# hellojialee/Improved-Body-Parts

Measured on AMD Instinct MI355X. Metric: fps_512_infer, higher is better.
Workload: dtype bf16; 1 GPU; model=4-stage IMHN @512x512, mode=infer, global_batch=4, input=512, parallelism=dp1

## Files before the change

### improved_body_parts_amd/models/layers.py

```python
from __future__ import annotations

import torch
import torch.nn.functional as F
from torch import nn

from .. import ops

LEAKY_SLOPE = 0.01


class Conv(nn.Module):

    def __init__(self, inp_dim, out_dim, kernel_size=3, stride=1, bn=True, relu=True,
                 dropout=False, dialated=1):
        super().__init__()
        self.inp_dim = inp_dim
        self.dropout = dropout
        self.relu = nn.LeakyReLU(negative_slope=LEAKY_SLOPE, inplace=True) if relu else None
        pad = (kernel_size - 1) // 2
        if bn:
            self.conv = nn.Conv2d(inp_dim, out_dim, kernel_size, stride, padding=pad, bias=False)
            self.bn = nn.BatchNorm2d(out_dim)
        else:
            self.conv = nn.Conv2d(inp_dim, out_dim, kernel_size, stride, padding=pad, bias=True)
# ... 76 lines not shown
        )
        if ins != outs:
            self.skipConv = nn.Sequential(
                nn.Conv2d(ins, outs, 1, bias=False),
                nn.BatchNorm2d(outs),
            )
        self.relu = nn.LeakyReLU(negative_slope=LEAKY_SLOPE, inplace=True)
        self.ins = ins
        self.outs = outs

    def forward(self, x):
        cb = self.convBlock
        y = ops.conv_bn_act(x, cb[0], cb[1], act=True, training=self.training)
        y = ops.conv_bn_act(y, cb[3], cb[4], act=True, training=self.training)
        if self.ins != self.outs:
            residual = ops.conv_bn_act(x, self.skipConv[0], self.skipConv[1], act=False,
                                       training=self.training)
        else:
            residual = x
        return ops.conv_bn_add_act(y, cb[6], cb[7], residual, act=self.relu_flag,
                                   training=self.training)


class BasicResidual(nn.Module):

    def __init__(self, inp_dim, out_dim, stride=1, bn=True, relu=True):
        super().__init__()
        self.relu_flag = relu
        self.conv1 = nn.Conv2d(inp_dim, out_dim, 3, padding=1, stride=stride, bias=False)
        self.bn1 = nn.BatchNorm2d(out_dim)
        self.relu1 = nn.LeakyReLU(negative_slope=LEAKY_SLOPE, inplace=True)
        self.conv2 = nn.Conv2d(out_dim, out_dim, 3, padding=1, bias=False)
        self.bn2 = nn.BatchNorm2d(out_dim)
        self.skip = nn.Sequential(
            nn.Conv2d(inp_dim, out_dim, 1, stride=stride, bias=False),
# ... 115 lines not shown
```

### improved_body_parts_amd/ops/__init__.py

```python
from __future__ import annotations

import os

import torch
import torch.nn.functional as F

from . import _backend
from ._backend import (
    hip_available,
    hip_extension,
    require_hip,
    use_hip_for,
)

LEAKY_SLOPE = 0.01



def conv_bn_act(x, conv, bn, act: bool, training: bool,
                residual_post=None, residual_post2=None):
    if use_hip_for(x):
        from . import conv as _conv
        return _conv.conv_bn_act_hip(x, conv, bn, act=act, residual=None,
                                     training=training,
# ... 27 lines not shown
                    residual_post=None):
    if use_hip_for(x):
        from . import conv as _conv
        return _conv.conv_bn_act_hip(x, conv, bn, act=act, residual=residual,
                                     training=training,
                                     residual_post=residual_post)
    y = conv(x)
    if bn is not None:
        y = bn(y)
    y = y + residual
    if act:
        y = F.leaky_relu(y, LEAKY_SLOPE, inplace=True)
    if residual_post is not None:
        y = y + residual_post
    return y


def conv_bn_act_group(items):
    if items and all(use_hip_for(it["x"]) for it in items):
        from . import conv as _conv
        return _conv.conv_bn_act_group_hip(items)
    out = []
    for it in items:
        if it.get("residual") is not None:
            y = conv_bn_add_act(
                it["x"], it["conv"], it["bn"], it["residual"], act=it["act"],
                training=it.get("training", False),
                residual_post=it.get("residual_post"))
            if it.get("residual_post2") is not None:
                y = y + it["residual_post2"]
# ... 105 lines not shown
```

### improved_body_parts_amd/ops/conv.py

```python
from __future__ import annotations

import os

import torch
import torch.nn.functional as F

from . import conv_kernels
from ._backend import hip_extension
from ._cache import versioned

LEAKY_SLOPE = 0.01
_CL = torch.channels_last


def _to_cl(t):
    return t.contiguous(memory_format=_CL)


def _conv_forward(x, weight, bias, stride, padding, dilation):
    y = conv_kernels.conv_fwd(x, weight, stride, padding, dilation)
    if y is None:
        y = F.conv2d(x, weight, None, stride, padding, dilation)
        y = _to_cl(y)
    if bias is not None:
# ... 220 lines not shown
def upsample_conv_bn_act_hip(low, conv, bn, act: bool, training: bool = False,
                             residual_post=None, residual_post2=None):
    if _on_inference_path(low, bn, training) and upconv_fold_enabled():
        if conv_kernels.upfold_supported(low, conv.weight, conv.stride,
                                         conv.padding, conv.dilation):
            scale, shift = _inference_epilogue(conv, bn)
            return conv_kernels.upfold_fwd(
                _to_cl(low), conv.weight, scale=scale, shift=shift, act=act,
                residual_post=residual_post, residual_post2=residual_post2)
    from . import spatial
    return conv_bn_act_hip(spatial.upsample2x_hip(low), conv, bn, act=act,
                           training=training, residual_post=residual_post,
                           residual_post2=residual_post2)


def conv_group_enabled() -> bool:
    return os.environ.get("IBP_CONV_GROUP", "1") != "0"


def conv_bn_act_group_hip(items):
    if len(items) > 1 and conv_group_enabled() and all(
            _on_inference_path(it["x"], it["bn"], it.get("training", False))
            for it in items):
        members = []
        for it in items:
            conv = it["conv"]
            scale, shift = _inference_epilogue(conv, it["bn"])
            members.append(dict(
                x=_to_cl(it["x"]), weight=conv.weight, stride=conv.stride,
                padding=conv.padding, dilation=conv.dilation, scale=scale,
# ... 13 lines not shown
```

### improved_body_parts_amd/ops/conv_kernels.py

```python
from __future__ import annotations

import os

import torch

from ._backend import hip_extension
from ._cache import versioned

_CL = torch.channels_last

DISABLE = os.environ.get("IBP_AMD_DISABLE_MFMA_CONV") == "1"


def _supported(x, stride):
    return not DISABLE and x.dtype == torch.bfloat16 \
        and stride[0] == stride[1]


def _cl(t):
    return None if t is None else t.contiguous(memory_format=_CL)


_NO_EPI = (None, None, None, False, None, None)

# ... 207 lines not shown
    cout = weight.shape[0]
    post = []
    for r in (residual_post, residual_post2):
        if r is not None:
            assert tuple(r.shape) == (n, cout, 2 * h, 2 * w_), \
                f"residual {tuple(r.shape)} is not the upsampled output shape"
            r = _cl(r).permute(0, 2, 3, 1)
        post.append(r)
    geom = [n, h, w_, cin, cout, 3, 3, 1, 1, 1, 1, 1, 2 * h, 2 * w_, 1]
    y = hip_extension().conv_mfma_upfold_fwd(
        x.permute(0, 2, 3, 1), upfold_packed_weight(weight), geom, scale,
        shift, act, *post)
    return y.permute(0, 3, 1, 2)


def conv_dgrad(dy, weight, x_shape, stride, padding, dilation):
    if not _supported(dy, stride):
        return None
    cout, _, kh, kw = weight.shape
    pad = (dilation[0] * (kh - 1) - padding[0],
           dilation[1] * (kw - 1) - padding[1])
    if pad[0] < 0 or pad[1] < 0:
        return None
    dx = hip_extension().conv_mfma_fwd(*_conv_args(
        dy, packed_weight_dgrad(weight), (x_shape[1], cout, kh, kw), (1, 1),
        pad, dilation, zs=stride[0], out_hw=x_shape[2:]))
    return dx.permute(0, 3, 1, 2)


def conv_wgrad(x, dy, w_shape, stride, padding, dilation):
# ... 6 lines not shown
```

### improved_body_parts_amd/ops/csrc/bindings.cpp

```cpp
#include <torch/extension.h>

using torch::Tensor;

std::vector<int64_t> bn_v8_geometry(int64_t M, int64_t C);
std::vector<Tensor> bn_stats(const Tensor& x_mc, int64_t C);
std::vector<Tensor> bn_finalize(
    const Tensor& sums, const Tensor& sumsq, int64_t M, const Tensor& gamma,
    const Tensor& beta, const c10::optional<Tensor>& running_mean,
    const c10::optional<Tensor>& running_var,
    const c10::optional<Tensor>& num_batches, double momentum, double eps);
std::vector<Tensor> bn_stats_finalize(
    const Tensor& x_mc, int64_t C, const Tensor& gamma, const Tensor& beta,
    const c10::optional<Tensor>& running_mean,
    const c10::optional<Tensor>& running_var,
    const c10::optional<Tensor>& num_batches, double momentum, double eps);
Tensor bn_act_fwd(const Tensor& x, const Tensor& scale, const Tensor& shift,
                  const c10::optional<Tensor>& residual, double slope, bool act);
std::vector<Tensor> bn_act_bwd(const Tensor& dy, const Tensor& y, const Tensor& x,
                               const c10::optional<Tensor>& mean,
                               const c10::optional<Tensor>& invstd,
                               double slope, bool act, bool need_xhat, int64_t C);
Tensor bn_act_bwd_apply(const Tensor& dpre, const Tensor& x, const Tensor& mean,
                        const Tensor& invstd, const Tensor& gamma,
                        const c10::optional<Tensor>& sum_dpre,
// ... 21 lines not shown

Tensor focal_l2_fwd(const Tensor& pred, const Tensor& gt, const Tensor& mask,
                    int64_t heat_start, int64_t bkg_start, int64_t gamma,
                    double mtw, double ktw, double alpha, double beta);
Tensor focal_l2_bwd(const Tensor& pred, const Tensor& gt, const Tensor& mask,
                    const Tensor& stack_gscale, int64_t heat_start,
                    int64_t bkg_start, int64_t gamma, double mtw, double ktw,
                    double alpha, double beta);

Tensor conv_mfma_fwd(const Tensor& x, const Tensor& w_packed,
                     const std::vector<int64_t>& geom,
                     const c10::optional<Tensor>& scale,
                     const c10::optional<Tensor>& shift,
                     const c10::optional<Tensor>& residual, bool act,
                     const c10::optional<Tensor>& residual_post,
                     const c10::optional<Tensor>& residual_post2);

std::vector<Tensor> conv_mfma_fwd_grouped(
    const std::vector<Tensor>& xs, const std::vector<Tensor>& ws_packed,
    const std::vector<std::vector<int64_t>>& geom,
    const std::vector<c10::optional<Tensor>>& scales,
    const std::vector<c10::optional<Tensor>>& shifts,
    const std::vector<c10::optional<Tensor>>& residuals,
    const std::vector<bool>& acts,
    const std::vector<c10::optional<Tensor>>& residual_posts,
    const std::vector<c10::optional<Tensor>>& residual_post2s);

std::vector<int64_t> conv_mfma_tile_plan(int64_t M, int64_t Cout, int64_t K);

void pack_conv_weight(const Tensor& w, Tensor& fwd_pack,
                      const c10::optional<Tensor>& dgrad_pack);

void pack_upfold_weight(const Tensor& w, Tensor& out);
Tensor conv_mfma_upfold_fwd(const Tensor& x_low, const Tensor& packs,
                            const std::vector<int64_t>& geom,
                            const c10::optional<Tensor>& scale,
                            const c10::optional<Tensor>& shift, bool act,
                            const c10::optional<Tensor>& residual_post,
                            const c10::optional<Tensor>& residual_post2);
std::vector<int64_t> conv_mfma_upfold_plan(int64_t M_low, int64_t Cout,
                                           int64_t Cin);

Tensor conv_mfma_wgrad(const Tensor& x, const Tensor& dy, int64_t N, int64_t H,
                       int64_t W, int64_t Cin, int64_t Cout, int64_t KH,
                       int64_t KW, int64_t stride, int64_t pad_h, int64_t pad_w,
                       int64_t dil_h, int64_t dil_w, int64_t Ho, int64_t Wo);
std::vector<int64_t> conv_wgrad_plan(int64_t M, int64_t Cin, int64_t Cout,
                                     int64_t KH, int64_t KW);
// ... 44 lines not shown
  m.def("upsample2x_bwd", &upsample2x_bwd);
  m.def("se_reduce", &se_reduce);
  m.def("se_scale", &se_scale);
  m.def("se_gate", &se_gate, "fused GAP-gate: sigmoid(W2@leaky(W1@p+b1)+b2)",
        py::arg("pooled"), py::arg("w1"), py::arg("b1"), py::arg("w2"),
        py::arg("b2"), py::arg("slope"), py::arg("pool_scale") = 1.0);
  m.def("se_layer_grouped", &se_layer_grouped,
        "inference SE layers of independent maps: one launch per stage");
  m.def("focal_l2_fwd", &focal_l2_fwd);
  m.def("focal_l2_bwd", &focal_l2_bwd);
  m.def("conv_mfma_fwd", &conv_mfma_fwd, "MFMA implicit-GEMM conv forward",
        py::arg("x"), py::arg("w_packed"), py::arg("geom"),
        py::arg("scale") = c10::nullopt, py::arg("shift") = c10::nullopt,
        py::arg("residual") = c10::nullopt, py::arg("act") = false,
        py::arg("residual_post") = c10::nullopt,
        py::arg("residual_post2") = c10::nullopt);
  m.def("conv_mfma_fwd_grouped", &conv_mfma_fwd_grouped,
        "independent MFMA convs in one grouped launch per 8 (+ one combine)",
        py::arg("xs"), py::arg("ws_packed"), py::arg("geom"),
        py::arg("scales"), py::arg("shifts"), py::arg("residuals"),
        py::arg("acts"), py::arg("residual_posts"),
        py::arg("residual_post2s"));
  m.def("conv_mfma_tile_plan", &conv_mfma_tile_plan,
        "debug: [BM, BN, splitk, deep] planned for GEMM extents (M, Cout, K)",
        py::arg("M"), py::arg("Cout"), py::arg("K"));
  m.def("pack_conv_weight", &pack_conv_weight,
        "fwd + dgrad weight packs in one kernel",
        py::arg("w"), py::arg("fwd_pack"), py::arg("dgrad_pack") = c10::nullopt);
  m.def("pack_upfold_weight", &pack_upfold_weight,
        "3x3 weight -> four folded 2x2 packs [4][Cout][4*Cin] (nearest-x2 "
        "upsample folded into the conv)",
        py::arg("w"), py::arg("out"));
  m.def("conv_mfma_upfold_fwd", &conv_mfma_upfold_fwd,
        "conv3x3(nearest_x2(x_low)) + epilogue as four parity 2x2 convs in "
        "one grouped launch",
        py::arg("x_low"), py::arg("packs"), py::arg("geom"),
        py::arg("scale") = c10::nullopt, py::arg("shift") = c10::nullopt,
        py::arg("act") = false, py::arg("residual_post") = c10::nullopt,
        py::arg("residual_post2") = c10::nullopt);
  m.def("conv_mfma_upfold_plan", &conv_mfma_upfold_plan,
        "debug: [BM, BN, splitk, deep] shared by the four parities of an "
        "upfold conv over M_low low-resolution pixels",
        py::arg("M_low"), py::arg("Cout"), py::arg("Cin"));
  m.def("conv_mfma_wgrad", &conv_mfma_wgrad,
        "MFMA implicit-GEMM conv weight gradient (tr16 LDS transpose)");
  m.def("conv_wgrad_plan", &conv_wgrad_plan,
        "debug: [TKD, TCO, waves, elem, kd_cb, chunks, chunk_len, tree group "
// ... 33 lines not shown
```

### improved_body_parts_amd/ops/csrc/conv_mfma.hip

```cpp
#include <torch/extension.h>
#include <ATen/hip/HIPContext.h>
#include <algorithm>
#include <type_traits>
#include <vector>
#include "common.h"
#include "conv_params.h"
#include "conv_plan.h"

namespace ibp {

typedef short short8 __attribute__((ext_vector_type(8)));
typedef float floatx4 __attribute__((ext_vector_type(4)));
typedef float floatx2 __attribute__((ext_vector_type(2)));
typedef unsigned short ushortv8 __attribute__((ext_vector_type(8)));
typedef unsigned short ushortv4 __attribute__((ext_vector_type(4)));

__device__ __forceinline__ int lds_off(int row, int k) {
  return row * BK + (k ^ ((row & 7) << 3));
}

template <int BM, int BN, bool DEEP, bool UP, typename Params>
__device__ __forceinline__ void conv_mfma_body(const Params& p,
                                               const int bid,
                                               unsigned short* lds_a,
                                               unsigned short* lds_b) {
  const int tid = threadIdx.x;
  const int lane = tid & 63;
  const int wave = tid >> 6;

  const int ntiles_n = (p.Cout + BN - 1) / BN;
  const int sk = bid % p.splitk;
  const int tile = bid / p.splitk;
  const int mt = tile / ntiles_n;
  const int nt = tile % ntiles_n;
  const long long m0 = (long long)mt * BM;
  const int n0 = nt * BN;
// ... 41 lines not shown
  const int hi_base = a_ho * p.stride - p.pad_h;
  const int wi_base = a_wo * p.stride - p.pad_w;

  const int nk_total = (p.K + BK - 1) / BK;
  const int nk_chunk = (nk_total + p.splitk - 1) / p.splitk;
  const int k_begin = sk * nk_chunk;
  const int nk = min(nk_chunk, nk_total - k_begin);
  if (nk <= 0) return;

  unsigned short a_reg0[A_ELEMS];
  unsigned short b_reg0[B_ELEMS];
  unsigned short a_reg1[A_ELEMS];
  unsigned short b_reg1[B_ELEMS];

  int t_kk = k_begin * BK + a_off;
  int t_f = t_kk / p.Cin;
  int t_ci = t_kk - t_f * p.Cin;
  int t_kh = t_f / p.KW;
  int t_kw = t_f - t_kh * p.KW;
  auto tap_advance = [&](int& ci, int& kh, int& kw, int step) {
    ci += step;
    while (ci >= p.Cin) {
      ci -= p.Cin;
      if (++kw == p.KW) { kw = 0; ++kh; }
    }
  };

  auto load_chunk = [&](int ck, unsigned short (&a_reg)[A_ELEMS],
                        unsigned short (&b_reg)[B_ELEMS]) {
    int kk = t_kk, ci = t_ci, kh = t_kh, kw = t_kw;
    if (ci + A_ELEMS <= p.Cin && kk + A_ELEMS <= p.K && p.zs == 1) {
      const int hi = hi_base + kh * p.dil_h;
      const int wi = wi_base + kw * p.dil_w;
      const bool ok = a_valid_row && hi >= 0 && hi < p.H &&
                      wi >= 0 && wi < p.W;
      const unsigned short* src =
          p.x + (((long long)a_n * p.H + hi) * p.W + wi) * p.Cin + ci;
      const bool aligned = ((reinterpret_cast<uintptr_t>(src)) & 15u) == 0;
      if (ok && aligned) {
        #pragma unroll
        for (int v = 0; v < A_ELEMS / 8; ++v)
          *reinterpret_cast<ushortv8*>(&a_reg[v * 8]) =
              *reinterpret_cast<const ushortv8*>(src + v * 8);
      } else if (ok) {
        #pragma unroll
// ... 46 lines not shown
          dst[e] = v;
          if (++cie == p.Cin) {
            cie = 0;
            if (++kwe == p.KW) { kwe = 0; ++khe; }
          }
        }
      } else {
        #pragma unroll
        for (int e = 0; e < 8; ++e) dst[e] = 0;
      }
      kk += 8;
      tap_advance(ci, kh, kw, 8);
    }
a_done:
    t_kk += BK;
    tap_advance(t_ci, t_kh, t_kw, BK);
    {
      int col = n0 + b_row;
      int kk = ck * BK + b_off;
      bool ok = col < p.Cout;
      const unsigned short* src = p.w + (long long)col * p.K + kk;
      bool b_aligned = ((reinterpret_cast<uintptr_t>(src)) & 15u) == 0;
      if (ok && b_aligned && kk + B_ELEMS <= p.K) {
        #pragma unroll
        for (int v = 0; v < B_ELEMS / 8; ++v)
          *reinterpret_cast<ushortv8*>(&b_reg[v * 8]) =
              *reinterpret_cast<const ushortv8*>(src + v * 8);
      } else {
        #pragma unroll
        for (int e = 0; e < B_ELEMS; ++e)
          b_reg[e] = (ok && kk + e < p.K) ? src[e] : 0;
// ... 232 lines not shown
          ws_slice[lin] = acc[i][j][r];
          continue;
        }
        const long long idx = out_idx(i, col + r, lin);
        float v = acc[i][j][r] * sc + sh;
        if (p.res) v += us2f(p.res[idx]);
        if (p.act) v = leaky(v, 0.01f);
        if (p.res_post) v += us2f(p.res_post[idx]);
        if (p.res_post2) v += us2f(p.res_post2[idx]);
        p.y[idx] = f2us(v);
      }
    }
  }
}

template <int BM, int BN, bool DEEP = false>
__global__ __launch_bounds__(256, 2) void conv_mfma_kernel(ConvParams p) {
  __shared__ unsigned short lds_a[2 * BM * BK];
  __shared__ unsigned short lds_b[2 * BN * BK];
  conv_mfma_body<BM, BN, DEEP, false>(p, blockIdx.x, lds_a, lds_b);
}

template <bool UP>
__global__ __launch_bounds__(256, 2) void conv_mfma_grouped_kernel(
    ConvGroupParams g) {
  __shared__ __attribute__((aligned(16))) unsigned short lds[4 * 128 * BK];
  const int gb = blockIdx.x;
  int pi = 0, base = 0, cfg = g.cfg[0];
  #pragma unroll
  for (int i = 0; i < kMaxGroup - 1; ++i) {
    if (i + 1 < g.n && gb >= g.block_end[i]) {
      pi = i + 1;
      base = g.block_end[i];
      cfg = g.cfg[i + 1];
    }
  }
  typedef __attribute__((address_space(4))) const char* kernarg_bytes;
  kernarg_bytes ka = (kernarg_bytes)__builtin_amdgcn_kernarg_segment_ptr();
  typedef __attribute__((address_space(4))) const ConvParams* kernarg_params;
  const auto& p = *(kernarg_params)(ka + offsetof(ConvGroupParams, p) +
                                    (size_t)pi * sizeof(ConvParams));
  const int bid = gb - base;
  switch (cfg) {
    case tile_cfg(128, 128, false):
      conv_mfma_body<128, 128, false, UP>(p, bid, lds, lds + 2 * 128 * BK); break;
    case tile_cfg(128, 128, true):
      conv_mfma_body<128, 128, true, UP>(p, bid, lds, lds + 2 * 128 * BK); break;
    case tile_cfg(128, 64, false):
      conv_mfma_body<128, 64, false, UP>(p, bid, lds, lds + 2 * 128 * BK); break;
    case tile_cfg(128, 64, true):
      conv_mfma_body<128, 64, true, UP>(p, bid, lds, lds + 2 * 128 * BK); break;
    case tile_cfg(64, 64, false):
      conv_mfma_body<64, 64, false, UP>(p, bid, lds, lds + 2 * 64 * BK); break;
    case tile_cfg(64, 64, true):
      conv_mfma_body<64, 64, true, UP>(p, bid, lds, lds + 2 * 64 * BK); break;
    case tile_cfg(32, 64, false):
      conv_mfma_body<32, 64, false, UP>(p, bid, lds, lds + 2 * 32 * BK); break;
    default:
      conv_mfma_body<32, 64, true, UP>(p, bid, lds, lds + 2 * 32 * BK); break;
  }
}

static_assert(std::is_same<decltype(&conv_mfma_grouped_kernel<false>),
                           void (*)(ConvGroupParams)>::value &&
                  std::is_same<decltype(&conv_mfma_grouped_kernel<true>),
                               void (*)(ConvGroupParams)>::value,
              "conv_mfma_grouped_kernel must take the table as its only "
              "argument: it is read at kernarg offset 0");

__device__ __forceinline__ float combine_one(float v, float sc, float sh,
                                             bool has_scale, bool has_res,
                                             float r0, int act, bool has_rp,
                                             float r1, bool has_rp2, float r2) {
  if (has_scale) v = v * sc + sh;
// ... 139 lines not shown
    long long t = i / Cin;
    const int tap = (int)(t & 3); t >>= 2;
    const int co = (int)(t % Cout);
    const int par = (int)(t / Cout);
    const int py = par >> 1, px = par & 1, a = tap >> 1, b = tap & 1;
    const int kh_lo = py == 0 ? a : 2 * a, kh_hi = py == 0 ? 2 * a : a + 1;
    const int kw_lo = px == 0 ? b : 2 * b, kw_hi = px == 0 ? 2 * b : b + 1;
    const unsigned short* src = w + ((long long)co * Cin + ci) * 9;
    float acc = 0.f;
    for (int kh = kh_lo; kh <= kh_hi; ++kh)
      for (int kw = kw_lo; kw <= kw_hi; ++kw) acc += us2f(src[kh * 3 + kw]);
    out[i] = f2us(acc);
  }
}

__global__ void pack_weight_kernel(const unsigned short* __restrict__ w,
                                   unsigned short* __restrict__ fwd,
                                   unsigned short* __restrict__ dgr,
                                   int Cout, int Cin, int KH, int KW) {
  const long long total = (long long)Cout * Cin * KH * KW;
  const int KHW = KH * KW;
  for (long long i = blockIdx.x * (long long)blockDim.x + threadIdx.x;
       i < total; i += (long long)gridDim.x * blockDim.x) {
    const int kw = (int)(i % KW);
    long long t = i / KW;
    const int kh = (int)(t % KH); t /= KH;
    const int ci = (int)(t % Cin);
    const int co = (int)(t / Cin);
    const unsigned short v = w[i];
    const int f = kh * KW + kw;
// ... 31 lines not shown
void pack_upfold_weight(const Tensor& w, Tensor& out) {
  TORCH_CHECK(w.is_cuda() && w.is_contiguous() && w.dim() == 4 &&
              w.scalar_type() == at::ScalarType::BFloat16 &&
              w.size(2) == 3 && w.size(3) == 3,
              "pack_upfold_weight: contiguous bf16 [Cout][Cin][3][3]");
  TORCH_CHECK(out.is_cuda() && out.is_contiguous() &&
              out.scalar_type() == at::ScalarType::BFloat16 &&
              out.numel() == 16 * w.size(0) * w.size(1),
              "pack_upfold_weight: out must be bf16 [4][Cout][4*Cin]");
  auto stream = at::hip::getCurrentHIPStream().stream();
  dim3 grid(ibp::grid_1d(out.numel(), 256, 2048)), block(256);
  hipLaunchKernelGGL(ibp::pack_upfold_weight_kernel, grid, block, 0, stream,
                     reinterpret_cast<const unsigned short*>(w.data_ptr()),
                     reinterpret_cast<unsigned short*>(out.data_ptr()),
                     (int)w.size(0), (int)w.size(1));
}

namespace {

using ibp::ConvPlan;
using ibp::ConvProblem;

const unsigned short* bf16_ptr(const OptTensor& t) {
  if (!t.has_value()) return nullptr;
  TORCH_CHECK(t->is_cuda() && t->scalar_type() == at::ScalarType::BFloat16,
              "conv_mfma: residuals must be bf16 device tensors");
  return reinterpret_cast<const unsigned short*>(t->data_ptr());
}

ConvProblem make_problem(const Tensor& x, const Tensor& w_packed,
// ... 11 lines not shown
  int* const row[15] = {&p.N, &p.H, &p.W, &p.Cin, &p.Cout, &p.KH, &p.KW,
                        &p.stride, &p.pad_h, &p.pad_w, &p.dil_h, &p.dil_w,
                        &p.Ho, &p.Wo, &p.zs};
  for (int i = 0; i < 15; ++i) *row[i] = (int)geom[i];
  p.x = reinterpret_cast<const unsigned short*>(x.data_ptr());
  p.w = reinterpret_cast<const unsigned short*>(w_packed.data_ptr());
  p.scale = scale.has_value() ? scale->data_ptr<float>() : nullptr;
  p.shift = shift.has_value() ? shift->data_ptr<float>() : nullptr;
  p.res = bf16_ptr(residual);
  p.res_post = bf16_ptr(residual_post);
  p.res_post2 = bf16_ptr(residual_post2);
  p.act = act ? 1 : 0;
  return q;
}

Tensor alloc_output(ConvProblem& q, const Tensor& x) {
  Tensor y = torch::empty({q.p.N, q.p.Ho, q.p.Wo, q.p.Cout}, x.options());
  q.p.y = reinterpret_cast<unsigned short*>(y.data_ptr());
  return y;
}

template <class F>
void with_flag(bool flag, F&& f) {
  if (flag) f(std::true_type{});
  else f(std::false_type{});
}

template <class F>
void with_tile(const ConvPlan& plan, F&& f) {
  using i128 = std::integral_constant<int, 128>;
  using i64 = std::integral_constant<int, 64>;
  using i32 = std::integral_constant<int, 32>;
  with_flag(plan.t.deep, [&](auto deep) {
    if (plan.t.BM == 128 && plan.t.BN == 128) f(i128{}, i128{}, deep);
    else if (plan.t.BM == 128) f(i128{}, i64{}, deep);
    else if (plan.t.BM == 64) f(i64{}, i64{}, deep);
    else f(i32{}, i64{}, deep);
  });
}

void launch_single(const ConvPlan& plan, hipStream_t stream) {
  const ibp::ConvParams& p = plan.p;
  TORCH_CHECK(!p.up, "upfold plans launch through the grouped kernel");
  with_tile(plan, [&](auto bm, auto bn, auto deep) {
    hipLaunchKernelGGL(
        (ibp::conv_mfma_kernel<decltype(bm)::value, decltype(bn)::value,
                               decltype(deep)::value>),
        dim3(plan.nblocks), dim3(256), 0, stream, p);
  });
  if (p.splitk > 1)
    with_flag(plan.vec_combine, [&](auto vec) {
      hipLaunchKernelGGL(ibp::splitk_combine_kernel<decltype(vec)::value>,
                         dim3(ibp::combine_blocks(plan)), dim3(256), 0, stream,
                         p.ws, p.y, p.scale, p.shift, p.res, p.res_post,
                         p.res_post2, (long long)p.M * p.Cout, p.Cout, p.act,
                         p.splitk);
    });
}

void launch_group(const ibp::GroupPlan& gp, hipStream_t stream) {
  with_flag(gp.up, [&](auto up) {
    hipLaunchKernelGGL(ibp::conv_mfma_grouped_kernel<decltype(up)::value>,
                       dim3(gp.blocks), dim3(256), 0, stream, gp.g);
// ... 20 lines not shown
      if (head.ws_elems > 0) ibp::set_workspace(head, workspace(head.ws_elems));
      launch_single(head, stream);
    } else {
      float* ws = workspace(ibp::group_workspace(plans, first, last));
      launch_group(ibp::assemble_group(plans, first, last, ws), stream);
    }
  }
}

}

Tensor conv_mfma_fwd(const Tensor& x, const Tensor& w_packed,
                     const std::vector<int64_t>& geom, const OptTensor& scale,
                     const OptTensor& shift, const OptTensor& residual,
                     bool act, const OptTensor& residual_post,
                     const OptTensor& residual_post2) {
  ConvProblem q = make_problem(x, w_packed, geom, scale, shift, residual, act,
                               residual_post, residual_post2);
  Tensor y = alloc_output(q, x);
  std::vector<ConvPlan> plans{ibp::plan_conv(q)};
  run_plans(plans, at::hip::getCurrentHIPStream().stream(),
            x.options().dtype(torch::kFloat32));
  return y;
}

std::vector<Tensor> conv_mfma_fwd_grouped(
    const std::vector<Tensor>& xs, const std::vector<Tensor>& ws_packed,
    const std::vector<std::vector<int64_t>>& geom,
    const std::vector<OptTensor>& scales, const std::vector<OptTensor>& shifts,
    const std::vector<OptTensor>& residuals, const std::vector<bool>& acts,
    const std::vector<OptTensor>& residual_posts,
    const std::vector<OptTensor>& residual_post2s) {
  const size_t n = xs.size();
// ... 79 lines not shown
```

### improved_body_parts_amd/ops/csrc/conv_params.h

```cpp
#pragma once

#include <cstddef>
#include <type_traits>

namespace ibp {

constexpr int BK = 64;

struct ConvParams {
  const unsigned short* x;
  const unsigned short* w;
  unsigned short* y;
  const float* scale;
  const float* shift;
  const unsigned short* res;
  const unsigned short* res_post;
  const unsigned short* res_post2;
  int N, H, W, Cin, Cout, KH, KW;
  int stride, pad_h, pad_w, dil_h, dil_w, Ho, Wo;
  int zs;
  long long M;
  int K;
  int n_mtiles;
  int act;
  int splitk;
  float* ws;
  int vec_epi;
  int pair_epi;
  int m32;
  int up, py, px;
};

constexpr int kMaxGroup = 8;

struct ConvGroupParams {
  ConvParams p[kMaxGroup];
  int block_end[kMaxGroup];
  int cfg[kMaxGroup];
  int n;
};

constexpr int tile_cfg(int BM, int BN, bool deep) {
  return ((BM == 128 ? (BN == 128 ? 0 : 1) : (BM == 64 ? 2 : 3)) << 1) |
         (deep ? 1 : 0);
}
// ... 34 lines not shown
```

### improved_body_parts_amd/ops/csrc/conv_plan.h

```cpp
#pragma once

#include <algorithm>
#include <cstdint>
#include <cstdlib>
#include <optional>
#include <stdexcept>
#include <string>
#include <vector>

#include "conv_params.h"

namespace ibp {

struct TilePlan {
  int BM, BN, n_mtiles, ntiles, splitk, nk_block;
  bool deep;
};

struct ConvProblem {
  ConvParams p{};
  std::optional<TilePlan> tile;
};

struct ConvPlan {
// ... 49 lines not shown

inline TilePlan plan_tile(long long M, int Cout, int K) {
  return plan_tiles(M, Cout, K, 1);
}

inline TilePlan plan_upfold_tile(long long M_low, int Cout, int Cin) {
  return plan_tiles(M_low, Cout, 4 * Cin, 4);
}

inline ConvPlan plan_conv(const ConvProblem& q) {
  ConvPlan plan;
  plan.p = q.p;
  ConvParams& p = plan.p;
  p.M = (long long)p.N * p.Ho * p.Wo;
  p.K = p.KH * p.KW * p.Cin;
  const TilePlan t = q.tile ? *q.tile : plan_tile(p.M, p.Cout, p.K);
  const int Cout = p.Cout, splitk = t.splitk;
  p.n_mtiles = t.n_mtiles;
  p.splitk = splitk;
  plan.ws_elems = splitk > 1 ? (long long)splitk * p.M * Cout : 0;
  p.ws = nullptr;
  p.vec_epi = Cout % 4 == 0 &&
              (splitk > 1 ||
               !(misaligned(p.scale, 16) || misaligned(p.shift, 16) ||
                 misaligned(p.res, 8) || misaligned(p.res_post, 8) ||
                 misaligned(p.res_post2, 8) || misaligned(p.y, 8)));
  if (p.vec_epi && Cout % 8 == 0 && !misaligned(p.y, 16)) p.vec_epi = 2;
  p.pair_epi = Cout % 2 == 0 &&
               !(misaligned(p.res, 4) || misaligned(p.res_post, 4) ||
                 misaligned(p.res_post2, 4) || misaligned(p.y, 4));
// ... 43 lines not shown
};

inline GroupPlan assemble_group(std::vector<ConvPlan>& plans, size_t first,
                                size_t last, float* ws_base) {
  const int n = (int)(last - first);
  if (n < 1 || n > kMaxGroup || last > plans.size())
    throw std::invalid_argument("grouped conv: 1 to kMaxGroup members");
  GroupPlan gp{};
  gp.up = plans[first].p.up != 0;
  long long ws_total = 0;
  for (int i = 0; i < n; ++i) {
    ConvPlan& plan = plans[first + i];
    if ((plan.p.up != 0) != gp.up)
      throw std::invalid_argument(
          "grouped conv: upfold and plain members cannot mix");
    gp.order[i] = i;
    gp.ws_off[i] = ws_total;
    if (plan.ws_elems > 0) set_workspace(plan, ws_base + ws_total);
    ws_total += ws_slice(plan);
  }
  std::stable_sort(gp.order, gp.order + n, [&](int a, int b) {
    return plans[first + a].t.nk_block > plans[first + b].t.nk_block;
  });
  for (int i = 0; i < kMaxGroup; ++i) {
    const ConvPlan& plan = plans[first + gp.order[i < n ? i : n - 1]];
    if (i < n) gp.blocks += plan.nblocks;
    gp.g.p[i] = plan.p;
    gp.g.cfg[i] = tile_cfg(plan.t.BM, plan.t.BN, plan.t.deep);
    gp.g.block_end[i] = gp.blocks;
  }
// ... 24 lines not shown
```

Before: 550.5 images/s.

## Fuse residual skip 1x1 conv into final 1x1 conv via K-concatenation

When a residual block's channel count changes, the final 1x1 conv+BN and the 1x1 skip conv+BN are merged into one GEMM. The two inputs are concatenated along K inside the MFMA kernel, and the BN scales are folded into one packed weight with a summed shift. This removes one kernel launch and the write and read of the intermediate residual tensor, at the cost of a new CAT kernel template variant and a weight pack that is cached per parameter version.

```diff
diff --git a/improved_body_parts_amd/models/layers.py b/improved_body_parts_amd/models/layers.py
--- a/improved_body_parts_amd/models/layers.py
+++ b/improved_body_parts_amd/models/layers.py
@@ -114,11 +114,10 @@
         y = ops.conv_bn_act(x, cb[0], cb[1], act=True, training=self.training)
         y = ops.conv_bn_act(y, cb[3], cb[4], act=True, training=self.training)
         if self.ins != self.outs:
-            residual = ops.conv_bn_act(x, self.skipConv[0], self.skipConv[1], act=False,
-                                       training=self.training)
-        else:
-            residual = x
-        return ops.conv_bn_add_act(y, cb[6], cb[7], residual, act=self.relu_flag,
+            return ops.conv_bn_add_conv_bn_act(
+                y, cb[6], cb[7], x, self.skipConv[0], self.skipConv[1],
+                act=self.relu_flag, training=self.training)
+        return ops.conv_bn_add_act(y, cb[6], cb[7], x, act=self.relu_flag,
                                    training=self.training)
 
 
diff --git a/improved_body_parts_amd/ops/__init__.py b/improved_body_parts_amd/ops/__init__.py
--- a/improved_body_parts_amd/ops/__init__.py
+++ b/improved_body_parts_amd/ops/__init__.py
@@ -65,6 +65,17 @@
     if residual_post is not None:
         y = y + residual_post
     return y
+
+
+def conv_bn_add_conv_bn_act(y, conv_a, bn_a, x, conv_b, bn_b, act: bool,
+                            training: bool):
+    if use_hip_for(y):
+        from . import conv as _conv
+        return _conv.conv_bn_add_conv_bn_act_hip(
+            y, conv_a, bn_a, x, conv_b, bn_b, act=act, training=training)
+    residual = conv_bn_act(x, conv_b, bn_b, act=False, training=training)
+    return conv_bn_add_act(y, conv_a, bn_a, residual, act=act,
+                           training=training)
 
 
 def conv_bn_act_group(items):
diff --git a/improved_body_parts_amd/ops/conv.py b/improved_body_parts_amd/ops/conv.py
--- a/improved_body_parts_amd/ops/conv.py
+++ b/improved_body_parts_amd/ops/conv.py
@@ -258,6 +258,61 @@
                            residual_post2=residual_post2)
 
 
+def skip_fold_enabled() -> bool:
+    return os.environ.get("IBP_SKIP_FOLD", "1") != "0"
+
+
+def _branch_fold(conv, bn):
+    if bn is not None and bn.weight is not None:
+        return _fold_bn(None, bn)
+    return None, (conv.bias.detach().float() if conv.bias is not None else None)
+
+
+def _fold_versions(conv, bn):
+    if bn is not None and bn.weight is not None:
+        return (conv.weight._version, bn.weight._version, bn.bias._version,
+                bn.running_mean._version, bn.running_var._version)
+    bias = conv.bias
+    return (conv.weight._version, bias._version if bias is not None else -1)
+
+
+def cat_fold(conv_a, bn_a, conv_b, bn_b):
+    wb = conv_b.weight
+    return versioned(conv_a.weight, ("cat", id(wb), id(bn_a), id(bn_b)),
+                     _fold_versions(conv_a, bn_a) + _fold_versions(conv_b, bn_b),
+                     _cat_build, conv_a, bn_a, conv_b, bn_b)[0]
+
+
+def _cat_build(prev, conv_a, bn_a, conv_b, bn_b):
+    scale_a, shift_a = _branch_fold(conv_a, bn_a)
+    scale_b, shift_b = _branch_fold(conv_b, bn_b)
+    packed = conv_kernels.cat_pack(prev[0] if prev is not None else None,
+                                   conv_a.weight, conv_b.weight, scale_a,
+                                   scale_b, shift_a, shift_b)
+    return packed, (conv_b.weight, bn_a, bn_b)
+
+
+def _plain_1x1(conv):
+    return (conv.kernel_size == (1, 1) and conv.stride == (1, 1)
+            and conv.padding == (0, 0) and conv.dilation == (1, 1)
+            and conv.groups == 1)
+
+
+def conv_bn_add_conv_bn_act_hip(y, conv_a, bn_a, x, conv_b, bn_b, act: bool,
+                                training: bool = False):
+    if skip_fold_enabled() and _on_inference_path(y, bn_a, training) \
+            and _on_inference_path(x, bn_b, training) \
+            and _plain_1x1(conv_a) and _plain_1x1(conv_b) \
+            and conv_kernels.cat_supported(y, conv_a.weight, x, conv_b.weight):
+        pack, ones, shift = cat_fold(conv_a, bn_a, conv_b, bn_b)
+        return conv_kernels.conv_cat_fwd(y, conv_a.weight, x, conv_b.weight,
+                                         pack, scale=ones, shift=shift,
+                                         act=act)
+    residual = conv_bn_act_hip(x, conv_b, bn_b, act=False, training=training)
+    return conv_bn_act_hip(y, conv_a, bn_a, act=act, residual=residual,
+                           training=training)
+
+
 def conv_group_enabled() -> bool:
     return os.environ.get("IBP_CONV_GROUP", "1") != "0"
 
diff --git a/improved_body_parts_amd/ops/conv_kernels.py b/improved_body_parts_amd/ops/conv_kernels.py
--- a/improved_body_parts_amd/ops/conv_kernels.py
+++ b/improved_body_parts_amd/ops/conv_kernels.py
@@ -245,6 +245,68 @@
     return y.permute(0, 3, 1, 2)
 
 
+
+def cat_weight_reference(wa, wb, scale_a=None, scale_b=None, shift_a=None,
+                         shift_b=None):
+    cout = wa.shape[0]
+    assert wb.shape[0] == cout and tuple(wa.shape[2:]) == (1, 1) \
+        and tuple(wb.shape[2:]) == (1, 1)
+    halves = []
+    for w, s in ((wa, scale_a), (wb, scale_b)):
+        h = w.detach().to(torch.bfloat16).float().reshape(cout, -1)
+        if s is not None:
+            h = h * s.detach().float().reshape(cout, 1)
+        halves.append(h.to(torch.bfloat16))
+    zero = torch.zeros(cout, dtype=torch.float32, device=wa.device)
+    shift = (zero if shift_a is None else shift_a.detach().float()) \
+        + (zero if shift_b is None else shift_b.detach().float())
+    return torch.cat(halves, dim=1).contiguous(), shift
+
+
+def cat_pack(prev, wa, wb, scale_a, scale_b, shift_a, shift_b):
+    cout = wa.shape[0]
+    k = wa.shape[1] + wb.shape[1]
+    wa, wb = wa.detach(), wb.detach()
+    if wa.is_cuda and wa.dtype == torch.bfloat16 and wb.dtype == wa.dtype:
+        if prev is not None:
+            pack, ones, shift = prev
+        else:
+            pack = torch.empty(cout, k, dtype=torch.bfloat16, device=wa.device)
+            ones = torch.ones(cout, dtype=torch.float32, device=wa.device)
+            shift = torch.empty(cout, dtype=torch.float32, device=wa.device)
+        hip_extension().pack_cat_weight(wa.contiguous(), wb.contiguous(),
+                                        scale_a, scale_b, shift_a, shift_b,
+                                        pack, shift)
+        return pack, ones, shift
+    pack, shift = cat_weight_reference(wa, wb, scale_a, scale_b, shift_a,
+                                       shift_b)
+    return pack, torch.ones_like(shift), shift
+
+
+def cat_supported(a, weight_a, b, weight_b) -> bool:
+    return (not DISABLE and a.is_cuda and b.is_cuda
+            and a.dtype == torch.bfloat16 and b.dtype == torch.bfloat16
+            and tuple(weight_a.shape[2:]) == (1, 1)
+            and tuple(weight_b.shape[2:]) == (1, 1)
+            and weight_a.shape[0] == weight_b.shape[0]
+            and a.shape[1] == weight_a.shape[1]
+            and b.shape[1] == weight_b.shape[1]
+            and weight_a.shape[1] % 64 == 0
+            and a.shape[0] == b.shape[0] and a.shape[2:] == b.shape[2:])
+
+
+def conv_cat_fwd(a, weight_a, b, weight_b, pack, scale=None, shift=None,
+                 act=False, residual_post=None, residual_post2=None):
+    a = a.contiguous(memory_format=_CL)
+    n, ca, h, w_ = a.shape
+    cout = weight_a.shape[0]
+    geom = [n, h, w_, ca, cout, 1, 1, 1, 0, 0, 1, 1, h, w_, 1]
+    y = hip_extension().conv_mfma_fwd(
+        a, pack, geom, scale, shift, None, bool(act), _cl(residual_post),
+        _cl(residual_post2), b.contiguous(memory_format=_CL))
+    return y.permute(0, 3, 1, 2)
+
+
 def conv_dgrad(dy, weight, x_shape, stride, padding, dilation):
     if not _supported(dy, stride):
         return None
diff --git a/improved_body_parts_amd/ops/csrc/bindings.cpp b/improved_body_parts_amd/ops/csrc/bindings.cpp
--- a/improved_body_parts_amd/ops/csrc/bindings.cpp
+++ b/improved_body_parts_amd/ops/csrc/bindings.cpp
@@ -59,7 +59,8 @@
                      const c10::optional<Tensor>& shift,
                      const c10::optional<Tensor>& residual, bool act,
                      const c10::optional<Tensor>& residual_post,
-                     const c10::optional<Tensor>& residual_post2);
+                     const c10::optional<Tensor>& residual_post2,
+                     const c10::optional<Tensor>& x2);
 
 std::vector<Tensor> conv_mfma_fwd_grouped(
     const std::vector<Tensor>& xs, const std::vector<Tensor>& ws_packed,
@@ -77,6 +78,12 @@
                       const c10::optional<Tensor>& dgrad_pack);
 
 void pack_upfold_weight(const Tensor& w, Tensor& out);
+void pack_cat_weight(const Tensor& wa, const Tensor& wb,
+                     const c10::optional<Tensor>& scale_a,
+                     const c10::optional<Tensor>& scale_b,
+                     const c10::optional<Tensor>& shift_a,
+                     const c10::optional<Tensor>& shift_b, Tensor& out,
+                     Tensor& shift_out);
 Tensor conv_mfma_upfold_fwd(const Tensor& x_low, const Tensor& packs,
                             const std::vector<int64_t>& geom,
                             const c10::optional<Tensor>& scale,
@@ -151,7 +158,8 @@
         py::arg("scale") = c10::nullopt, py::arg("shift") = c10::nullopt,
         py::arg("residual") = c10::nullopt, py::arg("act") = false,
         py::arg("residual_post") = c10::nullopt,
-        py::arg("residual_post2") = c10::nullopt);
+        py::arg("residual_post2") = c10::nullopt,
+        py::arg("x2") = c10::nullopt);
   m.def("conv_mfma_fwd_grouped", &conv_mfma_fwd_grouped,
         "independent MFMA convs in one grouped launch per 8 (+ one combine)",
         py::arg("xs"), py::arg("ws_packed"), py::arg("geom"),
@@ -168,6 +176,12 @@
         "3x3 weight -> four folded 2x2 packs [4][Cout][4*Cin] (nearest-x2 "
         "upsample folded into the conv)",
         py::arg("w"), py::arg("out"));
+  m.def("pack_cat_weight", &pack_cat_weight,
+        "two 1x1 weights (+ per-channel scales, shifts) -> one [Cout][Ca+Cb] "
+        "pack and the fused shift of a two-source 1x1 conv",
+        py::arg("wa"), py::arg("wb"), py::arg("scale_a"), py::arg("scale_b"),
+        py::arg("shift_a"), py::arg("shift_b"), py::arg("out"),
+        py::arg("shift_out"));
   m.def("conv_mfma_upfold_fwd", &conv_mfma_upfold_fwd,
         "conv3x3(nearest_x2(x_low)) + epilogue as four parity 2x2 convs in "
         "one grouped launch",
diff --git a/improved_body_parts_amd/ops/csrc/conv_mfma.hip b/improved_body_parts_amd/ops/csrc/conv_mfma.hip
--- a/improved_body_parts_amd/ops/csrc/conv_mfma.hip
+++ b/improved_body_parts_amd/ops/csrc/conv_mfma.hip
@@ -19,7 +19,7 @@
   return row * BK + (k ^ ((row & 7) << 3));
 }
 
-template <int BM, int BN, bool DEEP, bool UP, typename Params>
+template <int BM, int BN, bool DEEP, bool UP, bool CAT, typename Params>
 __device__ __forceinline__ void conv_mfma_body(const Params& p,
                                                const int bid,
                                                unsigned short* lds_a,
@@ -91,10 +91,13 @@
   unsigned short b_reg1[B_ELEMS];
 
   int t_kk = k_begin * BK + a_off;
-  int t_f = t_kk / p.Cin;
-  int t_ci = t_kk - t_f * p.Cin;
-  int t_kh = t_f / p.KW;
-  int t_kw = t_f - t_kh * p.KW;
+  int t_ci = 0, t_kh = 0, t_kw = 0;
+  if constexpr (!CAT) {
+    const int t_f = t_kk / p.Cin;
+    t_ci = t_kk - t_f * p.Cin;
+    t_kh = t_f / p.KW;
+    t_kw = t_f - t_kh * p.KW;
+  }
   auto tap_advance = [&](int& ci, int& kh, int& kw, int step) {
     ci += step;
     while (ci >= p.Cin) {
@@ -106,6 +109,25 @@
   auto load_chunk = [&](int ck, unsigned short (&a_reg)[A_ELEMS],
                         unsigned short (&b_reg)[B_ELEMS]) {
     int kk = t_kk, ci = t_ci, kh = t_kh, kw = t_kw;
+    if constexpr (CAT) {
+      const bool second = t_kk >= p.Cin;
+      const int C = second ? p.Cin2 : p.Cin;
+      const int c0 = second ? t_kk - p.Cin : t_kk;
+      const unsigned short* src =
+          (second ? p.x2 : p.x) + (long long)a_m * C + c0;
+      const bool aligned = ((reinterpret_cast<uintptr_t>(src)) & 15u) == 0;
+      if (a_valid_row && aligned && c0 + A_ELEMS <= C) {
+        #pragma unroll
+        for (int v = 0; v < A_ELEMS / 8; ++v)
+          *reinterpret_cast<ushortv8*>(&a_reg[v * 8]) =
+              *reinterpret_cast<const ushortv8*>(src + v * 8);
+      } else {
+        #pragma unroll
+        for (int e = 0; e < A_ELEMS; ++e)
+          a_reg[e] = (a_valid_row && c0 + e < C) ? src[e] : (unsigned short)0;
+      }
+      goto a_done;
+    }
     if (ci + A_ELEMS <= p.Cin && kk + A_ELEMS <= p.K && p.zs == 1) {
       const int hi = hi_base + kh * p.dil_h;
       const int wi = wi_base + kw * p.dil_w;
@@ -182,7 +204,7 @@
     }
 a_done:
     t_kk += BK;
-    tap_advance(t_ci, t_kh, t_kw, BK);
+    if constexpr (!CAT) tap_advance(t_ci, t_kh, t_kw, BK);
     {
       int col = n0 + b_row;
       int kk = ck * BK + b_off;
@@ -445,11 +467,11 @@
   }
 }
 
-template <int BM, int BN, bool DEEP = false>
+template <int BM, int BN, bool DEEP = false, bool CAT = false>
 __global__ __launch_bounds__(256, 2) void conv_mfma_kernel(ConvParams p) {
   __shared__ unsigned short lds_a[2 * BM * BK];
   __shared__ unsigned short lds_b[2 * BN * BK];
-  conv_mfma_body<BM, BN, DEEP, false>(p, blockIdx.x, lds_a, lds_b);
+  conv_mfma_body<BM, BN, DEEP, false, CAT>(p, blockIdx.x, lds_a, lds_b);
 }
 
 template <bool UP>
@@ -474,21 +496,21 @@
   const int bid = gb - base;
   switch (cfg) {
     case tile_cfg(128, 128, false):
-      conv_mfma_body<128, 128, false, UP>(p, bid, lds, lds + 2 * 128 * BK); break;
+      conv_mfma_body<128, 128, false, UP, false>(p, bid, lds, lds + 2 * 128 * BK); break;
     case tile_cfg(128, 128, true):
-      conv_mfma_body<128, 128, true, UP>(p, bid, lds, lds + 2 * 128 * BK); break;
+      conv_mfma_body<128, 128, true, UP, false>(p, bid, lds, lds + 2 * 128 * BK); break;
     case tile_cfg(128, 64, false):
-      conv_mfma_body<128, 64, false, UP>(p, bid, lds, lds + 2 * 128 * BK); break;
+      conv_mfma_body<128, 64, false, UP, false>(p, bid, lds, lds + 2 * 128 * BK); break;
     case tile_cfg(128, 64, true):
-      conv_mfma_body<128, 64, true, UP>(p, bid, lds, lds + 2 * 128 * BK); break;
+      conv_mfma_body<128, 64, true, UP, false>(p, bid, lds, lds + 2 * 128 * BK); break;
     case tile_cfg(64, 64, false):
-      conv_mfma_body<64, 64, false, UP>(p, bid, lds, lds + 2 * 64 * BK); break;
+      conv_mfma_body<64, 64, false, UP, false>(p, bid, lds, lds + 2 * 64 * BK); break;
     case tile_cfg(64, 64, true):
-      conv_mfma_body<64, 64, true, UP>(p, bid, lds, lds + 2 * 64 * BK); break;
+      conv_mfma_body<64, 64, true, UP, false>(p, bid, lds, lds + 2 * 64 * BK); break;
     case tile_cfg(32, 64, false):
-      conv_mfma_body<32, 64, false, UP>(p, bid, lds, lds + 2 * 32 * BK); break;
+      conv_mfma_body<32, 64, false, UP, false>(p, bid, lds, lds + 2 * 32 * BK); break;
     default:
-      conv_mfma_body<32, 64, true, UP>(p, bid, lds, lds + 2 * 32 * BK); break;
+      conv_mfma_body<32, 64, true, UP, false>(p, bid, lds, lds + 2 * 32 * BK); break;
   }
 }
 
@@ -658,6 +680,31 @@
   }
 }
 
+__global__ void pack_cat_weight_kernel(const unsigned short* __restrict__ wa,
+                                       const unsigned short* __restrict__ wb,
+                                       const float* __restrict__ scale_a,
+                                       const float* __restrict__ scale_b,
+                                       const float* __restrict__ shift_a,
+                                       const float* __restrict__ shift_b,
+                                       unsigned short* __restrict__ out,
+                                       float* __restrict__ shift_out,
+                                       int Cout, int Ca, int Cb) {
+  const int K = Ca + Cb;
+  const long long total = (long long)Cout * K;
+  for (long long i = blockIdx.x * (long long)blockDim.x + threadIdx.x;
+       i < total; i += (long long)gridDim.x * blockDim.x) {
+    const int k = (int)(i % K);
+    const int co = (int)(i / K);
+    const bool second = k >= Ca;
+    const unsigned short w = second ? wb[(long long)co * Cb + (k - Ca)]
+                                    : wa[(long long)co * Ca + k];
+    const float* scale = second ? scale_b : scale_a;
+    out[i] = f2us(us2f(w) * (scale ? scale[co] : 1.f));
+    if (i < Cout)
+      shift_out[i] = (shift_a ? shift_a[i] : 0.f) + (shift_b ? shift_b[i] : 0.f);
+  }
+}
+
 __global__ void pack_weight_kernel(const unsigned short* __restrict__ w,
                                    unsigned short* __restrict__ fwd,
                                    unsigned short* __restrict__ dgr,
@@ -719,6 +766,43 @@
                      reinterpret_cast<const unsigned short*>(w.data_ptr()),
                      reinterpret_cast<unsigned short*>(out.data_ptr()),
                      (int)w.size(0), (int)w.size(1));
+}
+
+void pack_cat_weight(const Tensor& wa, const Tensor& wb,
+                     const OptTensor& scale_a, const OptTensor& scale_b,
+                     const OptTensor& shift_a, const OptTensor& shift_b,
+                     Tensor& out, Tensor& shift_out) {
+  for (const Tensor* w : {&wa, &wb})
+    TORCH_CHECK(w->is_cuda() && w->is_contiguous() && w->dim() == 4 &&
+                w->scalar_type() == at::ScalarType::BFloat16 &&
+                w->size(2) == 1 && w->size(3) == 1 && w->size(0) == wa.size(0),
+                "pack_cat_weight: contiguous bf16 [Cout][C][1][1] weights "
+                "with equal Cout");
+  const int64_t Cout = wa.size(0), Ca = wa.size(1), Cb = wb.size(1);
+  TORCH_CHECK(out.is_cuda() && out.is_contiguous() &&
+              out.scalar_type() == at::ScalarType::BFloat16 &&
+              out.numel() == Cout * (Ca + Cb),
+              "pack_cat_weight: out must be bf16 [Cout][Ca+Cb]");
+  TORCH_CHECK(shift_out.is_cuda() && shift_out.is_contiguous() &&
+              shift_out.scalar_type() == at::ScalarType::Float &&
+              shift_out.numel() == Cout,
+              "pack_cat_weight: shift_out must be fp32 [Cout]");
+  auto vec = [&](const OptTensor& t) -> const float* {
+    if (!t.has_value()) return nullptr;
+    TORCH_CHECK(t->is_cuda() && t->is_contiguous() &&
+                t->scalar_type() == at::ScalarType::Float &&
+                t->numel() == Cout,
+                "pack_cat_weight: scales and shifts must be fp32 [Cout]");
+    return t->data_ptr<float>();
+  };
+  auto stream = at::hip::getCurrentHIPStream().stream();
+  dim3 grid(ibp::grid_1d(out.numel(), 256, 2048)), block(256);
+  hipLaunchKernelGGL(ibp::pack_cat_weight_kernel, grid, block, 0, stream,
+                     reinterpret_cast<const unsigned short*>(wa.data_ptr()),
+                     reinterpret_cast<const unsigned short*>(wb.data_ptr()),
+                     vec(scale_a), vec(scale_b), vec(shift_a), vec(shift_b),
+                     reinterpret_cast<unsigned short*>(out.data_ptr()),
+                     shift_out.data_ptr<float>(), (int)Cout, (int)Ca, (int)Cb);
 }
 
 namespace {
@@ -760,6 +844,25 @@
   return q;
 }
 
+void set_second_source(ConvProblem& q, const Tensor& x, const Tensor& x2,
+                       const Tensor& w_packed) {
+  ibp::ConvParams& p = q.p;
+  TORCH_CHECK(x2.is_cuda() && x2.device() == x.device() &&
+              x2.scalar_type() == at::ScalarType::BFloat16 && x2.dim() == 4 &&
+              x2.is_contiguous(at::MemoryFormat::ChannelsLast) &&
+              x2.size(0) == p.N && x2.size(2) == p.H && x2.size(3) == p.W,
+              "conv_mfma: x2 must be channels_last bf16 [N, Cin2, H, W]");
+  TORCH_CHECK(x.dim() == 4 &&
+              x.is_contiguous(at::MemoryFormat::ChannelsLast) &&
+              x.size(0) == p.N && x.size(1) == p.Cin && x.size(2) == p.H &&
+              x.size(3) == p.W,
+              "conv_mfma: with x2, x must be channels_last [N, Cin, H, W]");
+  p.Cin2 = (int)x2.size(1);
+  p.x2 = reinterpret_cast<const unsigned short*>(x2.data_ptr());
+  TORCH_CHECK(w_packed.numel() == (int64_t)p.Cout * (p.Cin + p.Cin2),
+              "conv_mfma: two-source pack must be [Cout][Cin + Cin2]");
+}
+
 Tensor alloc_output(ConvProblem& q, const Tensor& x) {
   Tensor y = torch::empty({q.p.N, q.p.Ho, q.p.Wo, q.p.Cout}, x.options());
   q.p.y = reinterpret_cast<unsigned short*>(y.data_ptr());
@@ -789,10 +892,12 @@
   const ibp::ConvParams& p = plan.p;
   TORCH_CHECK(!p.up, "upfold plans launch through the grouped kernel");
   with_tile(plan, [&](auto bm, auto bn, auto deep) {
-    hipLaunchKernelGGL(
-        (ibp::conv_mfma_kernel<decltype(bm)::value, decltype(bn)::value,
-                               decltype(deep)::value>),
-        dim3(plan.nblocks), dim3(256), 0, stream, p);
+    with_flag(p.Cin2 != 0, [&](auto cat) {
+      hipLaunchKernelGGL(
+          (ibp::conv_mfma_kernel<decltype(bm)::value, decltype(bn)::value,
+                                 decltype(deep)::value, decltype(cat)::value>),
+          dim3(plan.nblocks), dim3(256), 0, stream, p);
+    });
   });
   if (p.splitk > 1)
     with_flag(plan.vec_combine, [&](auto vec) {
@@ -843,9 +948,10 @@
                      const std::vector<int64_t>& geom, const OptTensor& scale,
                      const OptTensor& shift, const OptTensor& residual,
                      bool act, const OptTensor& residual_post,
-                     const OptTensor& residual_post2) {
+                     const OptTensor& residual_post2, const OptTensor& x2) {
   ConvProblem q = make_problem(x, w_packed, geom, scale, shift, residual, act,
                                residual_post, residual_post2);
+  if (x2.has_value()) set_second_source(q, x, *x2, w_packed);
   Tensor y = alloc_output(q, x);
   std::vector<ConvPlan> plans{ibp::plan_conv(q)};
   run_plans(plans, at::hip::getCurrentHIPStream().stream(),
diff --git a/improved_body_parts_amd/ops/csrc/conv_params.h b/improved_body_parts_amd/ops/csrc/conv_params.h
--- a/improved_body_parts_amd/ops/csrc/conv_params.h
+++ b/improved_body_parts_amd/ops/csrc/conv_params.h
@@ -29,6 +29,8 @@
   int pair_epi;
   int m32;
   int up, py, px;
+  int Cin2;
+  const unsigned short* x2;
 };
 
 constexpr int kMaxGroup = 8;
diff --git a/improved_body_parts_amd/ops/csrc/conv_plan.h b/improved_body_parts_amd/ops/csrc/conv_plan.h
--- a/improved_body_parts_amd/ops/csrc/conv_plan.h
+++ b/improved_body_parts_amd/ops/csrc/conv_plan.h
@@ -87,6 +87,26 @@
   ConvParams& p = plan.p;
   p.M = (long long)p.N * p.Ho * p.Wo;
   p.K = p.KH * p.KW * p.Cin;
+  if (p.x2 != nullptr || p.Cin2 != 0) {
+    if (p.x2 == nullptr || p.Cin2 <= 0)
+      throw std::invalid_argument(
+          "two-source conv: x2 and Cin2 > 0 go together");
+    if (p.Cin <= 0 || p.Cin % BK != 0)
+      throw std::invalid_argument(
+          "two-source conv: Cin must be a multiple of 64");
+    if (p.KH * p.KW != 1 || p.stride != 1 || p.pad_h != 0 || p.pad_w != 0 ||
+        p.dil_h != 1 || p.dil_w != 1 || p.zs != 1 || p.Ho != p.H ||
+        p.Wo != p.W)
+      throw std::invalid_argument(
+          "two-source conv: 1x1, stride 1, unpadded, undilated, zs 1 only");
+    if (p.up)
+      throw std::invalid_argument(
+          "two-source conv: cannot be an upfold parity");
+    if (q.tile)
+      throw std::invalid_argument(
+          "two-source conv: plans its own tile");
+    p.K = p.Cin + p.Cin2;
+  }
   const TilePlan t = q.tile ? *q.tile : plan_tile(p.M, p.Cout, p.K);
   const int Cout = p.Cout, splitk = t.splitk;
   p.n_mtiles = t.n_mtiles;
@@ -160,6 +180,9 @@
     if ((plan.p.up != 0) != gp.up)
       throw std::invalid_argument(
           "grouped conv: upfold and plain members cannot mix");
+    if (plan.p.Cin2 != 0)
+      throw std::invalid_argument(
+          "grouped conv: a two-source conv launches on its own");
     gp.order[i] = i;
     gp.ws_off[i] = ws_total;
     if (plan.ws_elems > 0) set_workspace(plan, ws_base + ws_total);
```

Measured after the change: 576.3 images/s, median of 6. 4.7% higher.
